# ADVRHumanoids/mpc_fatigue

Hardware: NVIDIA B200
Metric: rollout_steps_per_s_with_jacobians (higher is better)
Workload: dtype f64

## Files before the change

### mpc_fatigue_b200/csrc/kernels_jvp2.cu

```cuda
#include <atomic>
#include <cstdlib>
#include <mutex>
#include <vector>

#include "derivs.cuh"
#include "launch.cuh"

namespace mpcf {

template <int N>
struct WsLayout {
    static constexpr int kTile = 32;
    static constexpr int kPlanes2 = 3 * N * N;
    static constexpr int kPlanes1 = 4 * N;
    static constexpr int kQd = 0, kQdd = N, kFd = 2 * N, kQ = 3 * N;
    static constexpr int kStageDoubles = (kPlanes2 + kPlanes1) * kTile;
    static constexpr unsigned kStageBytes = kStageDoubles * sizeof(double);
    static constexpr int kRingDoubles = (kPlanes2 + 3 * N) * kTile;
    static constexpr unsigned kRingBytes = kRingDoubles * sizeof(double);
    static constexpr int kUnitDoubles = 4 * (kPlanes2 + kPlanes1);
    static MPCF_DI size_t chunk(long tile, int s) { return ((size_t)tile * 4 + s) * kStageDoubles; }
};
size_t jvp_ws_doubles_per_unit(int n) { return (size_t)4 * (3 * n * n + 4 * n); }

template <int N, int L>
__global__ void __launch_bounds__(kThreads) k_step_stages(const __grid_constant__ StaticParams<N> P, long U, long u0, long cnt,
                                                         const double *q, const double *qd, const double *tau, const double *theat,
                                                         long UT, const double *f, double dt, const double *dt_u, double *qn, double *qdn,
                                                         double *fn, double *ws)
{
    static_assert(N == L, "the pipeline runs one serial chain at a time (forests: one launch per chain)");
    const StaticModel<N, L> m{P};
    using D = Dyn<double, StaticModel<N, L>>;
    using W = WsLayout<N>;
    const long lu = (long)blockIdx.x * blockDim.x + threadIdx.x;
    if (lu >= cnt) return;
    const long u = u0 + lu;
    double x[3 * N], t[N], th[N], xs[3 * N], xn[3 * N], k[3 * N];
#pragma unroll
    for (int i = 0; i < N; ++i) {
        x[i] = q[i * U + u];
        x[N + i] = qd[i * U + u];
        x[2 * N + i] = f[i * U + u];
        t[i] = tau[i * U + u];
        th[i] = theat[i * UT + u];
    }
    const double h = dt_u ? dt_u[u] : dt;
#pragma unroll
    for (int i = 0; i < 3 * N; ++i) { xs[i] = x[i]; xn[i] = x[i]; }
#pragma unroll 1
    for (int s = 0; s < 4; ++s) {
        const double cs = s < 2 ? 0.5 : (s == 2 ? 1.0 : 0.0);
        const double wt = (s == 0 || s == 3) ? 1.0 / 6.0 : 1.0 / 3.0;
        double *w = ws + W::chunk(lu / 32, s) + W::kPlanes2 * 32 + (lu & 31);
        {
            double Cs[N * (N + 1) / 2];
            D::template fd_crba<L, true>(m, xs, xs + N, t, k + N, Cs);
#pragma unroll
            for (int i = 0; i < N; ++i) {
                k[i] = xs[N + i];
                k[2 * N + i] = D::fatigue_rhs(m, i, xs[2 * N + i], th[i], xs[N + i]);
            }
            double *c = ws + W::chunk(lu / 32, s) + 2 * N * N * 32 + (lu & 31);
#pragma unroll
            for (int r = 0; r < N; ++r)
#pragma unroll
                for (int cc = 0; cc < N; ++cc) __stcs(c + (r * N + cc) * 32, Cs[r >= cc ? r * (r + 1) / 2 + cc : cc * (cc + 1) / 2 + r]);
        }
#pragma unroll
        for (int i = 0; i < N; ++i) {
            __stcs(w + (W::kQ + i) * 32, xs[i]);
            __stcs(w + (W::kQd + i) * 32, xs[N + i]);
            __stcs(w + (W::kQdd + i) * 32, k[N + i]);
            __stcs(w + (W::kFd + i) * 32, k[2 * N + i]);
        }
        const double a = h * wt, c = h * cs;
#pragma unroll
        for (int i = 0; i < 3 * N; ++i) {
            xn[i] += a * k[i];
            xs[i] = x[i] + c * k[i];
        }
    }
    if (qn) {
#pragma unroll
        for (int i = 0; i < N; ++i) {
            qn[i * U + u] = xn[i];
            qdn[i * U + u] = xn[N + i];
            fn[i * U + u] = xn[2 * N + i];
        }
    }
}

constexpr int kSmCountHint = 148;
MPCF_DI void cp_async8(double *smem, const double *gmem)
{
    asm volatile("cp.async.ca.shared.global [%0], [%1], 8;" ::"r"((unsigned)__cvta_generic_to_shared(smem)), "l"(gmem) : "memory");
}
struct CFromShared {
    double *base;
    int stride;
    MPCF_DI void ready() const { asm volatile("cp.async.commit_group;\n\tcp.async.wait_group 0;" ::: "memory"); }
    MPCF_DI double operator()(int r, int c) const { return base[(r * (r + 1) / 2 + c) * stride]; }
};
template <int N>
struct CFromGlobal {
    const double *o;
    MPCF_DI void ready() const {}
    MPCF_DI double operator()(int r, int c) const { return o[(2 * N * N + r * N + c) * 32]; }
};

template <class F>
struct CFromRegisters {
    F f;
    MPCF_DI void ready() const {}
    MPCF_DI double operator()(int r, int c) const { return f(r, c); }
};

template <int N, int L, bool KSMEM>
__global__ void __launch_bounds__(kThreads) k_stage_derivs(const __grid_constant__ StaticParams<N> P, long cnt, double *ws)
{
    const StaticModel<N, L> m{P};
    using W = WsLayout<N>;
    const long lu = (long)blockIdx.x * blockDim.x + threadIdx.x;
    if (lu >= cnt) return;
    const int s = blockIdx.y;
    double *o = ws + W::chunk(lu / 32, s) + (lu & 31);
    const double *w = o + W::kPlanes2 * 32;
    double q[N], qd[N], qdd[N];
#pragma unroll
    for (int i = 0; i < N; ++i) {
        q[i] = __ldcs(w + (W::kQ + i) * 32);
        qd[i] = __ldcs(w + (W::kQd + i) * 32);
        qdd[i] = __ldcs(w + (W::kQdd + i) * 32);
    }
    {
        const long lin = (long)blockIdx.y * gridDim.x + blockIdx.x + 2 * kSmCountHint;
        if (lin < 4l * gridDim.x) {
            const long lu2 = (lin % gridDim.x) * blockDim.x + threadIdx.x;
            if (lu2 < cnt) {
                const double *o2 = ws + W::chunk(lu2 / 32, (int)(lin / gridDim.x)) + (lu2 & 31);
#pragma unroll
                for (int i = 0; i < N; ++i) {
                    asm volatile("prefetch.global.L2 [%0];" ::"l"(o2 + (W::kPlanes2 + W::kQ + i) * 32));
                    asm volatile("prefetch.global.L2 [%0];" ::"l"(o2 + (W::kPlanes2 + W::kQd + i) * 32));
                    asm volatile("prefetch.global.L2 [%0];" ::"l"(o2 + (W::kPlanes2 + W::kQdd + i) * 32));
                }
#pragma unroll
                for (int r = 0; r < N; ++r)
#pragma unroll
                    for (int c = 0; c <= r; ++c) asm volatile("prefetch.global.L2 [%0];" ::"l"(o2 + (2 * N * N + r * N + c) * 32));
            }
        }
    }
    auto emit = [&](int mat, int r, int c, double v) { __stcs(o + (mat * N * N + r * N + c) * 32, v); };
    if (KSMEM) {
        extern __shared__ double k2_slab[];
        SharedLinkStore ks{k2_slab + threadIdx.x, (int)blockDim.x};
        CFromShared Cs{k2_slab + 18 * (N - 1) * blockDim.x + threadIdx.x, (int)blockDim.x};
#pragma unroll
        for (int r = 0; r < N; ++r)
#pragma unroll
            for (int c = 0; c <= r; ++c) cp_async8(Cs.base + (r * (r + 1) / 2 + c) * Cs.stride, o + (2 * N * N + r * N + c) * 32);
        FdDerivs<StaticModel<N, L>, L>::run_cols(m, q, qd, qdd, Cs, emit, ks);
    } else {
        LocalLinkStore<N> ks;
        CFromGlobal<N> Cs{o};
        FdDerivs<StaticModel<N, L>, L>::run_cols(m, q, qd, qdd, Cs, emit, ks);
    }
}

template <int N>
__global__ void __launch_bounds__(kThreads) k_fd_derivs(const __grid_constant__ StaticParams<N> P, long U, const double *q, const double *qd,
                                                       const double *tau, double *Ao, double *Bo, double *Co, int ntot, int c0)
{
    const StaticModel<N, N> m{P};
    const long u = (long)blockIdx.x * blockDim.x + threadIdx.x;
    if (u >= U) return;
    double a[N], b[N], c[N], qdd[N], Cv[N * (N + 1) / 2];
#pragma unroll
    for (int i = 0; i < N; ++i) { a[i] = q[i * U + u]; b[i] = qd[i * U + u]; c[i] = tau[i * U + u]; }
    Dyn<double, StaticModel<N, N>>::template fd_crba<N, true>(m, a, b, c, qdd, Cv);
    auto at = [&](int r, int cc) { return (size_t)((c0 + r) * ntot + c0 + cc) * U + u; };
#pragma unroll
    for (int r = 0; r < N; ++r)
#pragma unroll
        for (int cc = 0; cc < N; ++cc) Co[at(r, cc)] = Cv[r >= cc ? r * (r + 1) / 2 + cc : cc * (cc + 1) / 2 + r];
    auto cget = [&](int r, int cc) { return Cv[r * (r + 1) / 2 + cc]; };
    CFromRegisters<decltype(cget)> Cs{cget};
    auto emit = [&](int mat, int r, int cc, double v) { (mat == 0 ? Ao : Bo)[at(r, cc)] = v; };
    extern __shared__ double link_slab[];
    SharedLinkStore ks{link_slab + threadIdx.x, (int)blockDim.x};
    FdDerivs<StaticModel<N, N>, N>::run_cols(m, a, b, qdd, Cs, emit, ks);
#pragma unroll 1
    for (int r = 0; r < N; ++r)
#pragma unroll 1
        for (int cc = 0; cc < ntot; ++cc)
            if (cc < c0 || cc >= c0 + N) {
                const size_t k = (size_t)((c0 + r) * ntot + cc) * U + u;
                Ao[k] = 0.0; Bo[k] = 0.0; Co[k] = 0.0;
            }
}

template <int N>
__global__ void __launch_bounds__(kThreads) k_rnea_derivs(const __grid_constant__ StaticParams<N> P, long U, const double *q, const double *qd,
                                                         const double *qdd, double *Dq, double *Dv, double *Mo, int ntot, int c0)
{
    const StaticModel<N, N> m{P};
    const long u = (long)blockIdx.x * blockDim.x + threadIdx.x;
    if (u >= U) return;
    double a[N], b[N], c[N];
#pragma unroll
    for (int i = 0; i < N; ++i) { a[i] = q[i * U + u]; b[i] = qd[i * U + u]; c[i] = qdd ? qdd[i * U + u] : 0.0; }
    extern __shared__ double link_slab[];
    SharedLinkStore ks{link_slab + threadIdx.x, (int)blockDim.x};
    struct Hooks {
        double *Dq, *Dv, *Mo;
        long U, u;
        int ntot, c0;
        MPCF_DI size_t at(int r, int cc) const { return (size_t)((c0 + r) * ntot + c0 + cc) * U + u; }
// ... 108 lines not shown
        for (int cc = 0; cc < ntot; ++cc)
            if (cc < c0 || cc >= c0 + N) { Dq[(size_t)((c0 + r) * ntot + cc) * U + u] = 0.0; Dv[(size_t)((c0 + r) * ntot + cc) * U + u] = 0.0; }
}

struct RneaDerivsDualBody {
    template <class MP>
    static MPCF_DI void run(const MP &m, long u, long U, const double *q, const double *qd, const double *qdd, double *Dq, double *Dv,
                            double *Mo)
    {
        constexpr int UNR = MP::kStatic ? MP::MAXN : 1;
        const int n = m.n();
        const int d = blockIdx.y;
        Dual a[MP::MAXN], b[MP::MAXN], c[MP::MAXN], t[MP::MAXN];
#pragma unroll UNR
        for (int i = 0; i < n; ++i) {
            a[i] = Dual(q[i * U + u], d == i ? 1.0 : 0.0);
            b[i] = Dual(qd[i * U + u], d == n + i ? 1.0 : 0.0);
            c[i] = Dual(qdd ? qdd[i * U + u] : 0.0, d == 2 * n + i ? 1.0 : 0.0);
        }
        Dyn<Dual, MP>::rnea(m, a, b, c, t);
        double *out = d < n ? Dq : (d < 2 * n ? Dv : Mo);
        const int col = d % n;
#pragma unroll UNR
        for (int r = 0; r < n; ++r) out[(size_t)(r * n + col) * U + u] = t[r].d;
    }
};

struct FdDerivsDualBody {
    template <class MP>
    static MPCF_DI void run(const MP &m, long u, long U, const double *q, const double *qd, const double *tau, double *Ao, double *Bo,
                            double *Co)
    {
        constexpr int UNR = MP::kStatic ? MP::MAXN : 1;
        const int n = m.n();
        const int d = blockIdx.y;
        Dual a[MP::MAXN], b[MP::MAXN], c[MP::MAXN], t[MP::MAXN];
#pragma unroll UNR
        for (int i = 0; i < n; ++i) {
            a[i] = Dual(q[i * U + u], d == i ? 1.0 : 0.0);
            b[i] = Dual(qd[i * U + u], d == n + i ? 1.0 : 0.0);
            c[i] = Dual(tau[i * U + u], d == 2 * n + i ? 1.0 : 0.0);
        }
        Dyn<Dual, MP>::aba(m, a, b, c, t);
        double *out = d < n ? Ao : (d < 2 * n ? Bo : Co);
        const int col = d % n;
#pragma unroll UNR
        for (int r = 0; r < n; ++r) out[(size_t)(r * n + col) * U + u] = t[r].d;
    }
};

template <int N, int L>
struct ColumnState {
    double Xq[N], Xv[N], Xf[N], aq[N], av[N], af[N];
    int jq, jv, jt;
    bool isdt;
    double ktau;
    double xq1;

    MPCF_DI void set_tau(const StaticParams<N> &P, double tauj)
    {
        ktau = 0.0;
#pragma unroll
        for (int i = 0; i < N; ++i)
            if (i == jt) ktau = 2.0 * P.fat[i][1] * P.fat[i][2] * tauj;
    }
    MPCF_DI void init(int col)
    {
        jq = col < N ? col : -1;
        jv = (col >= N && col < 2 * N) ? col - N : -1;
        jt = (col >= 2 * N && col < 3 * N) ? col - 2 * N : -1;
        isdt = col == 3 * N;
#pragma unroll
        for (int i = 0; i < N; ++i) {
            Xq[i] = (i == jq) ? 1.0 : 0.0;
            Xv[i] = (i == jv) ? 1.0 : 0.0;
            Xf[i] = 0.0;
            aq[i] = Xq[i]; av[i] = Xv[i]; af[i] = 0.0;
        }
        xq1 = 0.0;
    }
    MPCF_DI void finish(const StaticParams<N> &P, int s, const double *w1, double h, const double *nv)
    {
        const double cs = s < 2 ? 0.5 : (s == 2 ? 1.0 : 0.0);
        const double wt = (s == 0 || s == 3) ? 1.0 / 6.0 : 1.0 / 3.0;
#pragma unroll
        for (int i = 0; i < N; ++i) {
            const double qds = w1[(WsLayout<N>::kQd + i) * 32];
            double kf = 2.0 * P.fat[i][1] * P.fat[i][3] * qds * Xv[i] - P.fat[i][0] * Xf[i];
            if (i == jt) kf += ktau;
            double yq = h * Xv[i], yf = h * kf, yv = h * nv[i];
            if (isdt) {
                yq += qds;
                yv += w1[(WsLayout<N>::kQdd + i) * 32];
                yf += w1[(WsLayout<N>::kFd + i) * 32];
            }
            aq[i] = fma(wt, yq, aq[i]);
            av[i] = fma(wt, yv, av[i]);
            af[i] = fma(wt, yf, af[i]);
            Xq[i] = ((i == jq) ? 1.0 : 0.0) + cs * yq;
            Xv[i] = ((i == jv) ? 1.0 : 0.0) + cs * yv;
            Xf[i] = cs * yf;
            if (s == 0 && (i == jq || i == jv)) xq1 = Xq[i];
        }
    }
    MPCF_DI void stage(const StaticParams<N> &P, int s, const double *w, double h)
    {
        double nv[N];
        if (s == 0) {
#pragma unroll
            for (int r = 0; r < N; ++r) {
                double kv = 0.0;
                if (jq >= 0 && jq / L == r / L) kv = w[(r * N + jq) * 32];
                if (jv >= 0 && jv / L == r / L) kv = w[(N * N + r * N + jv) * 32];
                nv[r] = kv;
            }
        } else if (s == 1 && !isdt) {
            const int js = jq >= 0 ? jq : jv;
#pragma unroll
            for (int r = 0; r < N; ++r) {
                double kv = 0.0;
                if (js >= 0 && js / L == r / L) kv = w[(r * N + js) * 32] * xq1;
#pragma unroll
                for (int c = 0; c < N; ++c) {
                    if (r / L != c / L) continue;
                    kv = fma(w[(N * N + r * N + c) * 32], Xv[c], kv);
                }
                nv[r] = kv;
            }
        } else {
#pragma unroll
            for (int r = 0; r < N; ++r) {
                double kv = 0.0;
#pragma unroll
                for (int c = 0; c < N; ++c) {
                    if (r / L != c / L) continue;
                    kv = fma(w[(r * N + c) * 32], Xq[c], kv);
                    kv = fma(w[(N * N + r * N + c) * 32], Xv[c], kv);
                }
                nv[r] = kv;
            }
        }
        if (jt >= 0) {
#pragma unroll
            for (int r = 0; r < N; ++r)
                if (jt / L == r / L) nv[r] += w[(2 * N * N + r * N + jt) * 32];
        }
        finish(P, s, w + 3 * N * N * 32, h, nv);
    }
    static MPCF_DI void stage2(ColumnState &a, ColumnState &b, const StaticParams<N> &P, int s, const double *w, double h)
    {
        double na[N], nb[N];
#pragma unroll
        for (int r = 0; r < N; ++r) {
            double ka = 0.0, kb = 0.0;
#pragma unroll
            for (int c = 0; c < N; ++c) {
                if (r / L != c / L) continue;
                const double A = w[(r * N + c) * 32], B = w[(N * N + r * N + c) * 32];
                ka = fma(A, a.Xq[c], ka);
                kb = fma(A, b.Xq[c], kb);
                ka = fma(B, a.Xv[c], ka);
                kb = fma(B, b.Xv[c], kb);
            }
            if (a.jt >= 0 && a.jt / L == r / L) ka += w[(2 * N * N + r * N + a.jt) * 32];
            if (b.jt >= 0 && b.jt / L == r / L) kb += w[(2 * N * N + r * N + b.jt) * 32];
            na[r] = ka;
            nb[r] = kb;
        }
        a.finish(P, s, w + 3 * N * N * 32, h, na);
        b.finish(P, s, w + 3 * N * N * 32, h, nb);
    }
    template <bool WHOLE>
    MPCF_DI void store(const StaticParams<N> &P, int col, double h, long U, long u, double *jac, int ntot_, int c0_) const
    {
        const int ntot = WHOLE ? N : ntot_, c0 = WHOLE ? 0 : c0_;
        const long PC = 4 * ntot + 1;
        const long ocol = isdt ? 4 * ntot : (col / N) * ntot + c0 + col % N;
#pragma unroll
        for (int i = 0; i < N; ++i) {
            __stcs(jac + ((size_t)(c0 + i) * PC + ocol) * U + u, aq[i]);
            __stcs(jac + ((size_t)(ntot + c0 + i) * PC + ocol) * U + u, av[i]);
            __stcs(jac + ((size_t)(2 * ntot + c0 + i) * PC + ocol) * U + u, af[i]);
        }
        if (isdt) {
#pragma unroll
            for (int j = 0; j < N; ++j) {
                const double z = P.fat[j][0] * h;
                const double g = 1.0 + z * (-1.0 + z * (0.5 + z * (-1.0 / 6.0 + z * (1.0 / 24.0))));
                if (WHOLE) {
#pragma unroll
                    for (int r = 0; r < 3 * N; ++r) __stcs(jac + ((size_t)r * PC + 3 * N + j) * U + u, (r == 2 * N + j) ? g : 0.0);
                } else {
#pragma unroll
                    for (int blk = 0; blk < 3; ++blk)
#pragma unroll
                        for (int i = 0; i < N; ++i)
                            __stcs(jac + ((size_t)(blk * ntot + c0 + i) * PC + 3 * ntot + c0 + j) * U + u, (blk == 2 && i == j) ? g : 0.0);
                }
            }
        }
    }
};

MPCF_DI unsigned smem_u32(const void *p) { return (unsigned)__cvta_generic_to_shared(p); }
MPCF_DI void mbar_init(unsigned long long *bar, unsigned count)
{
    asm volatile("mbarrier.init.shared::cta.b64 [%0], %1;" ::"r"(smem_u32(bar)), "r"(count) : "memory");
}
MPCF_DI void mbar_arrive(unsigned long long *bar)
{
    asm volatile("{\n\t.reg .b64 st;\n\tmbarrier.arrive.shared::cta.b64 st, [%0];\n\t}" ::"r"(smem_u32(bar)) : "memory");
}
MPCF_DI void mbar_arrive_expect_tx(unsigned long long *bar, unsigned bytes)
{
    asm volatile("{\n\t.reg .b64 st;\n\tmbarrier.arrive.expect_tx.release.cta.shared::cta.b64 st, [%0], %1;\n\t}" ::"r"(smem_u32(bar)), "r"(bytes)
                 : "memory");
}
MPCF_DI void mbar_wait(unsigned long long *bar, unsigned parity)
{
    unsigned done;
    do {
        asm volatile("{\n\t.reg .pred p;\n\tmbarrier.try_wait.parity.shared::cta.b64 p, [%1], %2;\n\tselp.b32 %0, 1, 0, p;\n\t}"
                     : "=r"(done)
                     : "r"(smem_u32(bar)), "r"(parity)
                     : "memory");
    } while (!done);
}
MPCF_DI void bulk_g2s(void *dst, const void *src, unsigned bytes, unsigned long long *bar)
{
    asm volatile("cp.async.bulk.shared::cluster.global.mbarrier::complete_tx::bytes [%0], [%1], %2, [%3];" ::"r"(smem_u32(dst)), "l"(src),
                 "r"(bytes), "r"(smem_u32(bar))
                 : "memory");
}

template <class W, int NBUF>
MPCF_DI void tma_issue(unsigned item, double *buf, unsigned long long *full, unsigned long long *empty, const double *ws, unsigned bid,
                       unsigned nblk)
{
    const unsigned slot = item % NBUF, round = item / NBUF;
    const long t = bid + (long)(item / 4) * nblk;
    mbar_wait(&empty[slot], (round & 1) ^ 1);
    mbar_arrive_expect_tx(&full[slot], W::kRingBytes);
    bulk_g2s(buf + (size_t)slot * W::kRingDoubles, ws + W::chunk(t, item & 3), W::kRingBytes, &full[slot]);
}

template <int N, int L, int NBUF, int CPW, bool WHOLE>
__global__ void __launch_bounds__(32 * ((3 * N + CPW) / CPW), 1)
    k_chain_rule_tma(const __grid_constant__ StaticParams<N> P, long U, long u0, long cnt, const double *__restrict__ tau, long UT, double dt,
                     const double *__restrict__ dt_u, const double *__restrict__ ws, double *__restrict__ jac, long UJ, int ntot, int c0)
{
    using W = WsLayout<N>;
    constexpr int NC = 3 * N + 1;
    constexpr int NW = (NC + CPW - 1) / CPW;
    extern __shared__ __align__(128) unsigned char smem_raw[];
    double *buf = reinterpret_cast<double *>(smem_raw);
    unsigned long long *full = reinterpret_cast<unsigned long long *>(smem_raw + (size_t)NBUF * W::kRingBytes);
    unsigned long long *empty = full + NBUF;
    const int warp = threadIdx.x >> 5, lane = threadIdx.x & 31;
    const long ntiles = (cnt + 31) / 32;
    const long my_tiles = blockIdx.x < ntiles ? (ntiles - blockIdx.x + gridDim.x - 1) / gridDim.x : 0;
    const unsigned nitems = (unsigned)(my_tiles * 4);
    const bool producer = threadIdx.x == 0;
    if (producer) {
        for (int i = 0; i < NBUF; ++i) { mbar_init(&full[i], 1); mbar_init(&empty[i], NW); }
        asm volatile("fence.mbarrier_init.release.cluster;" ::: "memory");
        for (unsigned i = 0; i < NBUF - 1 && i < nitems; ++i)
            tma_issue<W, NBUF>(i, buf, full, empty, ws, blockIdx.x, gridDim.x);
    }
    __syncthreads();
    const int col0 = warp, col1 = warp + NW;
    const bool two = CPW == 2 && col1 < NC;
    unsigned it = 0;
    for (long t = blockIdx.x; t < ntiles; t += gridDim.x) {
        const long lu = t * 32 + lane;
        const bool live = lu < cnt;
        const long u = u0 + (live ? lu : 0);
        const double h = dt_u ? dt_u[u] : dt;
        ColumnState<N, L> a, b;
        a.init(col0);
        a.set_tau(P, a.jt >= 0 ? tau[(size_t)a.jt * UT + u] : 0.0);
        if (CPW == 2) {
            b.init(two ? col1 : col0);
            b.set_tau(P, b.jt >= 0 ? tau[(size_t)b.jt * UT + u] : 0.0);
        }
#pragma unroll 1
        for (int s = 0; s < 4; ++s, ++it) {
            if (producer && it + NBUF - 1 < nitems) tma_issue<W, NBUF>(it + NBUF - 1, buf, full, empty, ws, blockIdx.x, gridDim.x);
            const unsigned slot = it % NBUF, round = it / NBUF;
            mbar_wait(&full[slot], round & 1);
            const double *w = buf + (size_t)slot * W::kRingDoubles + lane;
            if (CPW == 2) ColumnState<N, L>::stage2(a, b, P, s, w, h);
            else a.stage(P, s, w, h);
            __syncwarp();
            if (lane == 0) mbar_arrive(&empty[slot]);
        }
        if (live) {
            a.template store<WHOLE>(P, col0, h, UJ, u, jac, ntot, c0);
            if (two) b.template store<WHOLE>(P, col1, h, UJ, u, jac, ntot, c0);
        }
    }
}

template <int N, int L, int NCY>
__global__ void __launch_bounds__(32 * NCY, 2)
    k_chain_rule_ldg(const __grid_constant__ StaticParams<N> P, long U, long u0, long cnt, const double *__restrict__ tau, long UT, double dt,
                     const double *__restrict__ dt_u, const double *__restrict__ ws, double *__restrict__ jac, long UJ, int ntot, int c0)
{
    using W = WsLayout<N>;
    const long lu = (long)blockIdx.x * 32 + threadIdx.x;
    if (lu >= cnt) return;
    const long u = u0 + lu;
    const double h = dt_u ? dt_u[u] : dt;
    constexpr int NC = 3 * N + 1;
    for (int col = threadIdx.y; col < NC; col += blockDim.y) {
        ColumnState<N, L> st;
        st.init(col);
        st.set_tau(P, st.jt >= 0 ? tau[(size_t)st.jt * UT + u] : 0.0);
#pragma unroll 1
        for (int s = 0; s < 4; ++s) st.stage(P, s, ws + W::chunk(blockIdx.x, s) + threadIdx.x, h);
        st.template store<false>(P, col, h, UJ, u, jac, ntot, c0);
    }
}

struct ProfEvent { cudaEvent_t a, b; int k; };
static std::atomic<bool> g_prof_on{false};
static std::mutex g_prof_mu;
static std::vector<ProfEvent> g_prof;
void jvp_profile_enable(bool on) { g_prof_on.store(on); }
static cudaEvent_t prof_begin(int k, cudaStream_t s)
{
    if (!g_prof_on.load(std::memory_order_relaxed)) return nullptr;
    ProfEvent e;
    cudaEventCreate(&e.a);
    cudaEventCreate(&e.b);
    e.k = k;
    cudaEventRecord(e.a, s);
    std::lock_guard<std::mutex> lk(g_prof_mu);
    g_prof.push_back(e);
    return e.b;
}
static void prof_end(cudaEvent_t b, cudaStream_t s)
{
    if (b) cudaEventRecord(b, s);
}
int jvp_profile_read(double *ms3, long *launches)
{
    std::lock_guard<std::mutex> lk(g_prof_mu);
    ms3[0] = ms3[1] = ms3[2] = 0.0;
    *launches = (long)g_prof.size();
    for (auto &e : g_prof) {
        float t = 0.f;
        cudaEventSynchronize(e.b);
        cudaEventElapsedTime(&t, e.a, e.b);
        ms3[e.k] += t;
        cudaEventDestroy(e.a);
        cudaEventDestroy(e.b);
    }
    g_prof.clear();
    return 0;
}

static int current_device()
{
    int dev = 0;
    cudaGetDevice(&dev);
    return dev >= 0 && dev < 64 ? dev : 0;
}
static int sm_count()
{
    static int n[64] = {};
    const int dev = current_device();
    if (!n[dev]) {
        cudaDeviceGetAttribute(&n[dev], cudaDevAttrMultiProcessorCount, dev);
        if (n[dev] <= 0) n[dev] = 148;
    }
    return n[dev];
}

template <int N, int L>
static cudaError_t run_jvp2(const StaticParams<N> &P, long U, long Ucnt, const double *q, const double *qd, const double *tau, const double *theat,
                            long UT, const double *f,
                            double dt, const double *dt_u, double *qn, double *qdn, double *fn, double *jac, long UJ, double *ws, long Uc,
                            cudaStream_t s, int ntot = N, int c0 = 0)
{
    using W = WsLayout<N>;
    constexpr bool kTma = N <= 7;
    constexpr int kRingMax = (227 * 1024 - 256) / (int)W::kRingBytes;
    constexpr int NBUF = kTma ? (kRingMax > 5 ? 5 : kRingMax) : 0;
    constexpr int kCpwDefault = (3 * N + 1 <= 19) ? 1 : 2;
    constexpr size_t smem = (size_t)NBUF * W::kRingBytes + 2 * NBUF * sizeof(unsigned long long);
    constexpr int kK2Threads = (2 * (18 * (N - 1) + N * (N + 1) / 2) * kThreads * (int)sizeof(double) <= 227 * 1024) ? kThreads : 96;
    constexpr int kK2Slab = (18 * (N - 1) + N * (N + 1) / 2) * kK2Threads * (int)sizeof(double);
    constexpr bool kK2Smem = N == L && 2 * kK2Slab <= 227 * 1024;
    if constexpr (kTma) {
        static std::atomic<bool> attr_set[64];
        const int dev = current_device();
        if (!attr_set[dev].load(std::memory_order_acquire)) {
            cudaError_t e = cudaSuccess;
            if constexpr (kCpwDefault == 1) {
                e = cudaFuncSetAttribute(k_chain_rule_tma<N, L, NBUF, 1, true>, cudaFuncAttributeMaxDynamicSharedMemorySize, (int)smem);
                if (e != cudaSuccess) return e;
                e = cudaFuncSetAttribute(k_chain_rule_tma<N, L, NBUF, 1, false>, cudaFuncAttributeMaxDynamicSharedMemorySize, (int)smem);
                if (e != cudaSuccess) return e;
            }
            e = cudaFuncSetAttribute(k_chain_rule_tma<N, L, NBUF, 2, true>, cudaFuncAttributeMaxDynamicSharedMemorySize, (int)smem);
            if (e != cudaSuccess) return e;
            e = cudaFuncSetAttribute(k_chain_rule_tma<N, L, NBUF, 2, false>, cudaFuncAttributeMaxDynamicSharedMemorySize, (int)smem);
            if (e != cudaSuccess) return e;
            if constexpr (kK2Smem) {
                e = cudaFuncSetAttribute(k_stage_derivs<N, L, true>, cudaFuncAttributeMaxDynamicSharedMemorySize, kK2Slab);
                if (e != cudaSuccess) return e;
            }
            attr_set[dev].store(true, std::memory_order_release);
        }
    }
    for (long u0 = 0; u0 < Ucnt; u0 += Uc) {
        const long cnt = (Ucnt - u0) < Uc ? (Ucnt - u0) : Uc;
        const unsigned gb = (unsigned)((cnt + kThreads - 1) / kThreads);
        const long ntiles = (cnt + 31) / 32;
        cudaEvent_t pe = prof_begin(0, s);
        k_step_stages<N, L><<<gb, kThreads, 0, s>>>(P, U, u0, cnt, q, qd, tau, theat, UT, f, dt, dt_u, qn, qdn, fn, ws);
        prof_end(pe, s);
        pe = prof_begin(1, s);
        static const int k2smem = getenv("MPCF_K2_SMEM") ? atoi(getenv("MPCF_K2_SMEM")) : 1;
        bool k2done = false;
        if constexpr (kK2Smem) {
            if (k2smem) {
                k_stage_derivs<N, L, true><<<dim3((unsigned)((cnt + kK2Threads - 1) / kK2Threads), 4), kK2Threads, kK2Slab, s>>>(P, cnt, ws);
                k2done = true;
            }
        }
        if (!k2done) k_stage_derivs<N, L, false><<<dim3(gb, 4), kThreads, 0, s>>>(P, cnt, ws);
        prof_end(pe, s);
        pe = prof_begin(2, s);
        if constexpr (kTma) {
            const unsigned g3 = (unsigned)(ntiles < sm_count() ? ntiles : sm_count());
            static const int cpw_env = getenv("MPCF_K3_CPW") ? atoi(getenv("MPCF_K3_CPW")) : 1;
            const int cpw = kCpwDefault == 2 ? 2 : cpw_env;
            if (cpw == 2) {
                (ntot == N ? k_chain_rule_tma<N, L, NBUF, 2, true> : k_chain_rule_tma<N, L, NBUF, 2, false>)<<<g3, 32 * ((3 * N + 2) / 2), smem, s>>>(
                    P, U, u0, cnt, theat, UT, dt, dt_u, ws, jac, UJ, ntot, c0);
            } else if constexpr (kCpwDefault == 1) {
                (ntot == N ? k_chain_rule_tma<N, L, NBUF, 1, true> : k_chain_rule_tma<N, L, NBUF, 1, false>)<<<g3, 32 * (3 * N + 1), smem, s>>>(
                    P, U, u0, cnt, theat, UT, dt, dt_u, ws, jac, UJ, ntot, c0);
            }
        } else {
            k_chain_rule_ldg<N, L, 10><<<(unsigned)ntiles, dim3(32, 10), 0, s>>>(P, U, u0, cnt, theat, UT, dt, dt_u, ws, jac, UJ, ntot, c0);
        }
        prof_end(pe, s);
        g_launches.fetch_add(3);
    }
    return cudaGetLastError();
}

template <int L, class V>
__global__ void __launch_bounds__(256) k_forest_fill_cross(int ntot, long cntv, long UJ, double *jac)
{
    const long uv = (long)blockIdx.x * blockDim.x + threadIdx.x;
    if (uv >= cntv) return;
    const int r = blockIdx.y, rc = (r % ntot) / L, nch = ntot / L;
    const long PC = 4 * ntot + 1;
    V zero;
    memset(&zero, 0, sizeof(V));
    double *row = jac + (size_t)r * PC * UJ;
    for (int b = 0; b < 4; ++b)
        for (int oc = 0; oc < nch; ++oc) {
            if (oc == rc) continue;
            double *p = row + (size_t)(b * ntot + oc * L) * UJ;
#pragma unroll
            for (int i = 0; i < L; ++i) __stcs(reinterpret_cast<V *>(p + (size_t)i * UJ) + uv, zero);
        }
}

template <int L>
static cudaError_t run_forest(const LaunchModel &m, long U, long Ucnt, const double *q, const double *qd, const double *tau, const double *theat,
                              long UT, const double *f, double dt,
                              const double *dt_u, double *qn, double *qdn, double *fn, double *jac, long UJ, double *ws, long Uc, cudaStream_t s)
{
    const StaticParams<L> *cp = static_cast<const StaticParams<L> *>(m.chain_params);
    for (int c = 0; c < m.n / L; ++c) {
        const size_t off = (size_t)c * L * U;
        cudaError_t e = run_jvp2<L, L>(cp[c], U, Ucnt, q + off, qd + off, tau + off, theat + (size_t)c * L * UT, UT, f + off, dt, dt_u, qn ? qn + off : nullptr,
                                       qdn ? qdn + off : nullptr, fn ? fn + off : nullptr, jac, UJ, ws, Uc, s, m.n, L * c);
        if (e != cudaSuccess) return e;
    }
    if (Ucnt % 2 == 0 && UJ % 2 == 0 && (reinterpret_cast<size_t>(jac) & 15) == 0)
        k_forest_fill_cross<L, double2><<<dim3((unsigned)((Ucnt / 2 + 255) / 256), 3 * m.n), 256, 0, s>>>(m.n, Ucnt / 2, UJ, jac);
    else
        k_forest_fill_cross<L, double><<<dim3((unsigned)((Ucnt + 255) / 256), 3 * m.n), 256, 0, s>>>(m.n, Ucnt, UJ, jac);
    g_launches.fetch_add(1);
    return cudaGetLastError();
}

bool jvp2_supported(const LaunchModel &m) { return family_chain_len(m.fam) > 0; }

cudaError_t launch_step_jvp_ws(const LaunchModel &m, long U, const double *q, const double *qd, const double *tau, const double *f,
                               double dt, const double *dt_u, double *qn, double *qdn, double *fn, double *jac, double *ws,
                               size_t ws_bytes, cudaStream_t s, long cnt, long UJ, const double *theat, long UT)
// ... 120 lines not shown
```

Baseline: 230.2 million.

## Swizzle workspace planes and stage Jacobian stores through shared memory

Adds an XOR swizzle on the per-tile workspace planes so lanes reading several planes from the shared-memory ring hit different banks, and routes all workspace accesses through the new layout. For one-column-per-warp chain-rule kernels it adds a specialised flat stage path plus a padded shared staging buffer with named barriers, so Jacobian outputs are transposed and written coalesced. The column-per-warp choice becomes compile-time by N, dropping the environment switch. This trades ring capacity for staging memory and adds barrier synchronisation among the worker warps.

```diff
diff --git a/mpc_fatigue_b200/csrc/kernels_jvp2.cu b/mpc_fatigue_b200/csrc/kernels_jvp2.cu
--- a/mpc_fatigue_b200/csrc/kernels_jvp2.cu
+++ b/mpc_fatigue_b200/csrc/kernels_jvp2.cu
@@ -1,6 +1,7 @@
 #include <atomic>
 #include <cstdlib>
 #include <mutex>
+#include <type_traits>
 #include <vector>
 
 #include "derivs.cuh"
@@ -20,6 +21,20 @@
     static constexpr unsigned kRingBytes = kRingDoubles * sizeof(double);
     static constexpr int kUnitDoubles = 4 * (kPlanes2 + kPlanes1);
     static MPCF_DI size_t chunk(long tile, int s) { return ((size_t)tile * 4 + s) * kStageDoubles; }
+    static MPCF_HD int swz(int plane) { return 4 * (plane % 3); }
+    static MPCF_HD int at(int plane, int u) { return plane * kTile + (u ^ swz(plane)); }
+};
+
+template <int N>
+struct WsView {
+    const double *b0, *b1, *b2;
+    MPCF_DI WsView(const double *chunk, int u) : b0(chunk + u), b1(chunk + (u ^ 4)), b2(chunk + (u ^ 8)) {}
+    MPCF_DI const double *ptr(int P) const
+    {
+        const int k = P % 3;
+        return (k == 0 ? b0 : (k == 1 ? b1 : b2)) + P * WsLayout<N>::kTile;
+    }
+    MPCF_DI double operator[](int P) const { return *ptr(P); }
 };
 size_t jvp_ws_doubles_per_unit(int n) { return (size_t)4 * (3 * n * n + 4 * n); }
 
@@ -52,7 +67,8 @@
     for (int s = 0; s < 4; ++s) {
         const double cs = s < 2 ? 0.5 : (s == 2 ? 1.0 : 0.0);
         const double wt = (s == 0 || s == 3) ? 1.0 / 6.0 : 1.0 / 3.0;
-        double *w = ws + W::chunk(lu / 32, s) + W::kPlanes2 * 32 + (lu & 31);
+        double *w = ws + W::chunk(lu / 32, s);
+        const int uu = (int)(lu & 31);
         {
             double Cs[N * (N + 1) / 2];
             D::template fd_crba<L, true>(m, xs, xs + N, t, k + N, Cs);
@@ -61,18 +77,18 @@
                 k[i] = xs[N + i];
                 k[2 * N + i] = D::fatigue_rhs(m, i, xs[2 * N + i], th[i], xs[N + i]);
             }
-            double *c = ws + W::chunk(lu / 32, s) + 2 * N * N * 32 + (lu & 31);
 #pragma unroll
             for (int r = 0; r < N; ++r)
 #pragma unroll
-                for (int cc = 0; cc < N; ++cc) __stcs(c + (r * N + cc) * 32, Cs[r >= cc ? r * (r + 1) / 2 + cc : cc * (cc + 1) / 2 + r]);
+                for (int cc = 0; cc < N; ++cc)
+                    __stcs(w + W::at(2 * N * N + r * N + cc, uu), Cs[r >= cc ? r * (r + 1) / 2 + cc : cc * (cc + 1) / 2 + r]);
         }
 #pragma unroll
         for (int i = 0; i < N; ++i) {
-            __stcs(w + (W::kQ + i) * 32, xs[i]);
-            __stcs(w + (W::kQd + i) * 32, xs[N + i]);
-            __stcs(w + (W::kQdd + i) * 32, k[N + i]);
-            __stcs(w + (W::kFd + i) * 32, k[2 * N + i]);
+            __stcs(w + W::at(W::kPlanes2 + W::kQ + i, uu), xs[i]);
+            __stcs(w + W::at(W::kPlanes2 + W::kQd + i, uu), xs[N + i]);
+            __stcs(w + W::at(W::kPlanes2 + W::kQdd + i, uu), k[N + i]);
+            __stcs(w + W::at(W::kPlanes2 + W::kFd + i, uu), k[2 * N + i]);
         }
         const double a = h * wt, c = h * cs;
 #pragma unroll
@@ -105,8 +121,9 @@
 template <int N>
 struct CFromGlobal {
     const double *o;
+    int u;
     MPCF_DI void ready() const {}
-    MPCF_DI double operator()(int r, int c) const { return o[(2 * N * N + r * N + c) * 32]; }
+    MPCF_DI double operator()(int r, int c) const { return o[WsLayout<N>::at(2 * N * N + r * N + c, u)]; }
 };
 
 template <class F>
@@ -124,35 +141,36 @@
     const long lu = (long)blockIdx.x * blockDim.x + threadIdx.x;
     if (lu >= cnt) return;
     const int s = blockIdx.y;
-    double *o = ws + W::chunk(lu / 32, s) + (lu & 31);
-    const double *w = o + W::kPlanes2 * 32;
+    double *o = ws + W::chunk(lu / 32, s);
+    const int uu = (int)(lu & 31);
     double q[N], qd[N], qdd[N];
 #pragma unroll
     for (int i = 0; i < N; ++i) {
-        q[i] = __ldcs(w + (W::kQ + i) * 32);
-        qd[i] = __ldcs(w + (W::kQd + i) * 32);
-        qdd[i] = __ldcs(w + (W::kQdd + i) * 32);
+        q[i] = __ldcs(o + W::at(W::kPlanes2 + W::kQ + i, uu));
+        qd[i] = __ldcs(o + W::at(W::kPlanes2 + W::kQd + i, uu));
+        qdd[i] = __ldcs(o + W::at(W::kPlanes2 + W::kQdd + i, uu));
     }
     {
         const long lin = (long)blockIdx.y * gridDim.x + blockIdx.x + 2 * kSmCountHint;
         if (lin < 4l * gridDim.x) {
             const long lu2 = (lin % gridDim.x) * blockDim.x + threadIdx.x;
             if (lu2 < cnt) {
-                const double *o2 = ws + W::chunk(lu2 / 32, (int)(lin / gridDim.x)) + (lu2 & 31);
+                const double *o2 = ws + W::chunk(lu2 / 32, (int)(lin / gridDim.x));
+                const int u2 = (int)(lu2 & 31);
 #pragma unroll
                 for (int i = 0; i < N; ++i) {
-                    asm volatile("prefetch.global.L2 [%0];" ::"l"(o2 + (W::kPlanes2 + W::kQ + i) * 32));
-                    asm volatile("prefetch.global.L2 [%0];" ::"l"(o2 + (W::kPlanes2 + W::kQd + i) * 32));
-                    asm volatile("prefetch.global.L2 [%0];" ::"l"(o2 + (W::kPlanes2 + W::kQdd + i) * 32));
+                    asm volatile("prefetch.global.L2 [%0];" ::"l"(o2 + W::at(W::kPlanes2 + W::kQ + i, u2)));
+                    asm volatile("prefetch.global.L2 [%0];" ::"l"(o2 + W::at(W::kPlanes2 + W::kQd + i, u2)));
+                    asm volatile("prefetch.global.L2 [%0];" ::"l"(o2 + W::at(W::kPlanes2 + W::kQdd + i, u2)));
                 }
 #pragma unroll
                 for (int r = 0; r < N; ++r)
 #pragma unroll
-                    for (int c = 0; c <= r; ++c) asm volatile("prefetch.global.L2 [%0];" ::"l"(o2 + (2 * N * N + r * N + c) * 32));
-            }
-        }
-    }
-    auto emit = [&](int mat, int r, int c, double v) { __stcs(o + (mat * N * N + r * N + c) * 32, v); };
+                    for (int c = 0; c <= r; ++c) asm volatile("prefetch.global.L2 [%0];" ::"l"(o2 + W::at(2 * N * N + r * N + c, u2)));
+            }
+        }
+    }
+    auto emit = [&](int mat, int r, int c, double v) { __stcs(o + W::at(mat * N * N + r * N + c, uu), v); };
     if (KSMEM) {
         extern __shared__ double k2_slab[];
         SharedLinkStore ks{k2_slab + threadIdx.x, (int)blockDim.x};
@@ -160,11 +178,11 @@
 #pragma unroll
         for (int r = 0; r < N; ++r)
 #pragma unroll
-            for (int c = 0; c <= r; ++c) cp_async8(Cs.base + (r * (r + 1) / 2 + c) * Cs.stride, o + (2 * N * N + r * N + c) * 32);
+            for (int c = 0; c <= r; ++c) cp_async8(Cs.base + (r * (r + 1) / 2 + c) * Cs.stride, o + W::at(2 * N * N + r * N + c, uu));
         FdDerivs<StaticModel<N, L>, L>::run_cols(m, q, qd, qdd, Cs, emit, ks);
     } else {
         LocalLinkStore<N> ks;
-        CFromGlobal<N> Cs{o};
+        CFromGlobal<N> Cs{o, uu};
         FdDerivs<StaticModel<N, L>, L>::run_cols(m, q, qd, qdd, Cs, emit, ks);
     }
 }
@@ -379,78 +397,78 @@
 template <int N, int L>
 struct ColumnState {
     double Xq[N], Xv[N], Xf[N], aq[N], av[N], af[N];
-    int jq, jv, jt;
-    bool isdt;
-    double ktau;
-    double xq1;
+    int col;
+    MPCF_DI int jq() const { return col < N ? col : -1; }
+    MPCF_DI int jv() const { return (col >= N && col < 2 * N) ? col - N : -1; }
+    MPCF_DI int jt() const { return (col >= 2 * N && col < 3 * N) ? col - 2 * N : -1; }
+    MPCF_DI bool isdt() const { return col == 3 * N; }
+    double aux;
 
     MPCF_DI void set_tau(const StaticParams<N> &P, double tauj)
     {
-        ktau = 0.0;
+        aux = 0.0;
 #pragma unroll
         for (int i = 0; i < N; ++i)
-            if (i == jt) ktau = 2.0 * P.fat[i][1] * P.fat[i][2] * tauj;
-    }
-    MPCF_DI void init(int col)
-    {
-        jq = col < N ? col : -1;
-        jv = (col >= N && col < 2 * N) ? col - N : -1;
-        jt = (col >= 2 * N && col < 3 * N) ? col - 2 * N : -1;
-        isdt = col == 3 * N;
+            if (i == jt()) aux = 2.0 * P.fat[i][1] * P.fat[i][2] * tauj;
+    }
+    MPCF_DI void init(int c)
+    {
+        col = c;
 #pragma unroll
         for (int i = 0; i < N; ++i) {
-            Xq[i] = (i == jq) ? 1.0 : 0.0;
-            Xv[i] = (i == jv) ? 1.0 : 0.0;
+            Xq[i] = (i == jq()) ? 1.0 : 0.0;
+            Xv[i] = (i == jv()) ? 1.0 : 0.0;
             Xf[i] = 0.0;
             aq[i] = Xq[i]; av[i] = Xv[i]; af[i] = 0.0;
         }
-        xq1 = 0.0;
-    }
-    MPCF_DI void finish(const StaticParams<N> &P, int s, const double *w1, double h, const double *nv)
-    {
+    }
+    template <bool NODT = false>
+    MPCF_DI void finish(const StaticParams<N> &P, int s, const WsView<N> &w, double h, const double *nv)
+    {
+        using W = WsLayout<N>;
         const double cs = s < 2 ? 0.5 : (s == 2 ? 1.0 : 0.0);
         const double wt = (s == 0 || s == 3) ? 1.0 / 6.0 : 1.0 / 3.0;
 #pragma unroll
         for (int i = 0; i < N; ++i) {
-            const double qds = w1[(WsLayout<N>::kQd + i) * 32];
+            const double qds = w[W::kPlanes2 + W::kQd + i];
             double kf = 2.0 * P.fat[i][1] * P.fat[i][3] * qds * Xv[i] - P.fat[i][0] * Xf[i];
-            if (i == jt) kf += ktau;
+            if (i == jt()) kf += aux;
             double yq = h * Xv[i], yf = h * kf, yv = h * nv[i];
-            if (isdt) {
+            if (!NODT && isdt()) {
                 yq += qds;
-                yv += w1[(WsLayout<N>::kQdd + i) * 32];
-                yf += w1[(WsLayout<N>::kFd + i) * 32];
+                yv += w[W::kPlanes2 + W::kQdd + i];
+                yf += w[W::kPlanes2 + W::kFd + i];
             }
             aq[i] = fma(wt, yq, aq[i]);
             av[i] = fma(wt, yv, av[i]);
             af[i] = fma(wt, yf, af[i]);
-            Xq[i] = ((i == jq) ? 1.0 : 0.0) + cs * yq;
-            Xv[i] = ((i == jv) ? 1.0 : 0.0) + cs * yv;
+            Xq[i] = ((i == jq()) ? 1.0 : 0.0) + cs * yq;
+            Xv[i] = ((i == jv()) ? 1.0 : 0.0) + cs * yv;
             Xf[i] = cs * yf;
-            if (s == 0 && (i == jq || i == jv)) xq1 = Xq[i];
-        }
-    }
-    MPCF_DI void stage(const StaticParams<N> &P, int s, const double *w, double h)
+            if (s == 0 && (i == jq() || i == jv())) aux = Xq[i];
+        }
+    }
+    MPCF_DI void stage(const StaticParams<N> &P, int s, const WsView<N> &w, double h)
     {
         double nv[N];
         if (s == 0) {
 #pragma unroll
             for (int r = 0; r < N; ++r) {
                 double kv = 0.0;
-                if (jq >= 0 && jq / L == r / L) kv = w[(r * N + jq) * 32];
-                if (jv >= 0 && jv / L == r / L) kv = w[(N * N + r * N + jv) * 32];
+                if (jq() >= 0 && jq() / L == r / L) kv = w[r * N + jq()];
+                if (jv() >= 0 && jv() / L == r / L) kv = w[N * N + r * N + jv()];
                 nv[r] = kv;
             }
-        } else if (s == 1 && !isdt) {
-            const int js = jq >= 0 ? jq : jv;
+        } else if (s == 1 && !isdt()) {
+            const int js = jq() >= 0 ? jq() : jv();
 #pragma unroll
             for (int r = 0; r < N; ++r) {
                 double kv = 0.0;
-                if (js >= 0 && js / L == r / L) kv = w[(r * N + js) * 32] * xq1;
+                if (js >= 0 && js / L == r / L) kv = w[r * N + js] * aux;
 #pragma unroll
                 for (int c = 0; c < N; ++c) {
                     if (r / L != c / L) continue;
-                    kv = fma(w[(N * N + r * N + c) * 32], Xv[c], kv);
+                    kv = fma(w[N * N + r * N + c], Xv[c], kv);
                 }
                 nv[r] = kv;
             }
@@ -461,20 +479,63 @@
 #pragma unroll
                 for (int c = 0; c < N; ++c) {
                     if (r / L != c / L) continue;
-                    kv = fma(w[(r * N + c) * 32], Xq[c], kv);
-                    kv = fma(w[(N * N + r * N + c) * 32], Xv[c], kv);
+                    kv = fma(w[r * N + c], Xq[c], kv);
+                    kv = fma(w[N * N + r * N + c], Xv[c], kv);
                 }
                 nv[r] = kv;
             }
         }
-        if (jt >= 0) {
+        if (jt() >= 0) {
 #pragma unroll
             for (int r = 0; r < N; ++r)
-                if (jt / L == r / L) nv[r] += w[(2 * N * N + r * N + jt) * 32];
-        }
-        finish(P, s, w + 3 * N * N * 32, h, nv);
-    }
-    static MPCF_DI void stage2(ColumnState &a, ColumnState &b, const StaticParams<N> &P, int s, const double *w, double h)
+                if (jt() / L == r / L) nv[r] += w[2 * N * N + r * N + jt()];
+        }
+        finish(P, s, w, h, nv);
+    }
+    MPCF_DI void stage_flat(const StaticParams<N> &P, int s, const double *slot, const WsView<N> &w, int lpA, double h)
+    {
+        static_assert(N == L && N % 3 == 0, "one serial chain with a plane count per row that keeps the swizzle class");
+        constexpr int T = WsLayout<N>::kTile, RS = N * T;
+        const int lp0 = lpA + (col / N) * (N * N * T), lpC = lpA + 2 * N * N * T;
+        const bool istau = jt() >= 0;
+        double nv[N];
+        if (s == 0) {
+#pragma unroll
+            for (int r = 0; r < N; ++r) {
+                const double e = slot[lp0 + r * RS];
+                nv[r] = istau ? 0.0 + e : e;
+            }
+        } else {
+            if (s == 1) {
+#pragma unroll
+                for (int r = 0; r < N; ++r) {
+                    const double e = slot[lpA + r * RS];
+                    double kv = istau ? 0.0 : e * aux;
+#pragma unroll
+                    for (int c = 0; c < N; ++c) kv = fma(w[N * N + r * N + c], Xv[c], kv);
+                    nv[r] = kv;
+                }
+            } else {
+#pragma unroll
+                for (int r = 0; r < N; ++r) {
+                    double kv = 0.0;
+#pragma unroll
+                    for (int c = 0; c < N; ++c) {
+                        kv = fma(w[r * N + c], Xq[c], kv);
+                        kv = fma(w[N * N + r * N + c], Xv[c], kv);
+                    }
+                    nv[r] = kv;
+                }
+            }
+#pragma unroll
+            for (int r = 0; r < N; ++r) {
+                const double e = istau ? slot[lpC + r * RS] : 0.0;
+                nv[r] = istau ? nv[r] + e : nv[r];
+            }
+        }
+        finish<true>(P, s, w, h, nv);
+    }
+    static MPCF_DI void stage2(ColumnState &a, ColumnState &b, const StaticParams<N> &P, int s, const WsView<N> &w, double h)
     {
         double na[N], nb[N];
 #pragma unroll
@@ -483,33 +544,33 @@
 #pragma unroll
             for (int c = 0; c < N; ++c) {
                 if (r / L != c / L) continue;
-                const double A = w[(r * N + c) * 32], B = w[(N * N + r * N + c) * 32];
+                const double A = w[r * N + c], B = w[N * N + r * N + c];
                 ka = fma(A, a.Xq[c], ka);
                 kb = fma(A, b.Xq[c], kb);
                 ka = fma(B, a.Xv[c], ka);
                 kb = fma(B, b.Xv[c], kb);
             }
-            if (a.jt >= 0 && a.jt / L == r / L) ka += w[(2 * N * N + r * N + a.jt) * 32];
-            if (b.jt >= 0 && b.jt / L == r / L) kb += w[(2 * N * N + r * N + b.jt) * 32];
+            if (a.jt() >= 0 && a.jt() / L == r / L) ka += w[2 * N * N + r * N + a.jt()];
+            if (b.jt() >= 0 && b.jt() / L == r / L) kb += w[2 * N * N + r * N + b.jt()];
             na[r] = ka;
             nb[r] = kb;
         }
-        a.finish(P, s, w + 3 * N * N * 32, h, na);
-        b.finish(P, s, w + 3 * N * N * 32, h, nb);
+        a.finish(P, s, w, h, na);
+        b.finish(P, s, w, h, nb);
     }
     template <bool WHOLE>
     MPCF_DI void store(const StaticParams<N> &P, int col, double h, long U, long u, double *jac, int ntot_, int c0_) const
     {
         const int ntot = WHOLE ? N : ntot_, c0 = WHOLE ? 0 : c0_;
         const long PC = 4 * ntot + 1;
-        const long ocol = isdt ? 4 * ntot : (col / N) * ntot + c0 + col % N;
+        const long ocol = isdt() ? 4 * ntot : (col / N) * ntot + c0 + col % N;
 #pragma unroll
         for (int i = 0; i < N; ++i) {
             __stcs(jac + ((size_t)(c0 + i) * PC + ocol) * U + u, aq[i]);
             __stcs(jac + ((size_t)(ntot + c0 + i) * PC + ocol) * U + u, av[i]);
             __stcs(jac + ((size_t)(2 * ntot + c0 + i) * PC + ocol) * U + u, af[i]);
         }
-        if (isdt) {
+        if (isdt()) {
 #pragma unroll
             for (int j = 0; j < N; ++j) {
                 const double z = P.fat[j][0] * h;
@@ -571,6 +632,14 @@
     bulk_g2s(buf + (size_t)slot * W::kRingDoubles, ws + W::chunk(t, item & 3), W::kRingBytes, &full[slot]);
 }
 
+template <int N>
+struct JacStage {
+    static constexpr int kPitch = 33;
+    static constexpr int kDoubles = N * 3 * N * kPitch;
+};
+
+MPCF_DI void named_bar_sync(int id, int threads) { asm volatile("bar.sync %0, %1;" ::"r"(id), "r"(threads) : "memory"); }
+
 template <int N, int L, int NBUF, int CPW, bool WHOLE>
 __global__ void __launch_bounds__(32 * ((3 * N + CPW) / CPW), 1)
     k_chain_rule_tma(const __grid_constant__ StaticParams<N> P, long U, long u0, long cnt, const double *__restrict__ tau, long UT, double dt,
@@ -579,9 +648,10 @@
     using W = WsLayout<N>;
     constexpr int NC = 3 * N + 1;
     constexpr int NW = (NC + CPW - 1) / CPW;
+    constexpr size_t kStgBytes = CPW == 1 ? JacStage<N>::kDoubles * sizeof(double) : 0;
     extern __shared__ __align__(128) unsigned char smem_raw[];
     double *buf = reinterpret_cast<double *>(smem_raw);
-    unsigned long long *full = reinterpret_cast<unsigned long long *>(smem_raw + (size_t)NBUF * W::kRingBytes);
+    unsigned long long *full = reinterpret_cast<unsigned long long *>(smem_raw + (size_t)NBUF * W::kRingBytes + kStgBytes);
     unsigned long long *empty = full + NBUF;
     const int warp = threadIdx.x >> 5, lane = threadIdx.x & 31;
     const long ntiles = (cnt + 31) / 32;
@@ -595,35 +665,87 @@
             tma_issue<W, NBUF>(i, buf, full, empty, ws, blockIdx.x, gridDim.x);
     }
     __syncthreads();
-    const int col0 = warp, col1 = warp + NW;
-    const bool two = CPW == 2 && col1 < NC;
     unsigned it = 0;
-    for (long t = blockIdx.x; t < ntiles; t += gridDim.x) {
-        const long lu = t * 32 + lane;
-        const bool live = lu < cnt;
-        const long u = u0 + (live ? lu : 0);
-        const double h = dt_u ? dt_u[u] : dt;
-        ColumnState<N, L> a, b;
-        a.init(col0);
-        a.set_tau(P, a.jt >= 0 ? tau[(size_t)a.jt * UT + u] : 0.0);
-        if (CPW == 2) {
+    if constexpr (CPW == 1) {
+        constexpr int NF = 3 * N;
+        constexpr int SP = JacStage<N>::kPitch;
+        double *stg = buf + (size_t)NBUF * W::kRingDoubles;
+        auto tiles = [&](auto dt_warp) {
+            constexpr bool DTW = decltype(dt_warp)::value;
+            const int uo = DTW ? lane : (int)threadIdx.x / NF;
+            const int col = DTW ? NF : (int)threadIdx.x % NF;
+            const int j = col % N;
+            const int lpA = W::at(j, uo);
+            for (long t = blockIdx.x; t < ntiles; t += gridDim.x) {
+                const long lu = t * 32 + uo;
+                const bool live = lu < cnt;
+                const long u = u0 + (live ? lu : 0);
+                const double h = dt_u ? dt_u[u] : dt;
+                ColumnState<N, L> a;
+                a.init(col);
+                a.set_tau(P, a.jt() >= 0 ? tau[(size_t)a.jt() * UT + u] : 0.0);
+#pragma unroll 1
+                for (int s = 0; s < 4; ++s, ++it) {
+                    if (producer && it + NBUF - 1 < nitems) tma_issue<W, NBUF>(it + NBUF - 1, buf, full, empty, ws, blockIdx.x, gridDim.x);
+                    const unsigned slot = it % NBUF, round = it / NBUF;
+                    mbar_wait(&full[slot], round & 1);
+                    const double *w = buf + (size_t)slot * W::kRingDoubles;
+                    if (DTW) a.stage(P, s, WsView<N>(w, uo), h);
+                    else a.stage_flat(P, s, w, WsView<N>(w, uo), lpA, h);
+                    __syncwarp();
+                    if (lane == 0) mbar_arrive(&empty[slot]);
+                }
+                if (DTW) {
+                    if (live) a.template store<WHOLE>(P, col, h, UJ, u, jac, ntot, c0);
+                    continue;
+                }
+                const int nt = WHOLE ? N : ntot, cz = WHOLE ? 0 : c0;
+                const int PC = 4 * nt + 1;
+                const int ocol = (warp / N) * nt + cz + warp % N;
+                const bool out = t * 32 + lane < cnt;
+                double *dst = jac + (u0 + t * 32 + lane);
+#pragma unroll
+                for (int blk = 0; blk < 3; ++blk) {
+                    named_bar_sync(1, 32 * NF);
+#pragma unroll
+                    for (int i = 0; i < N; ++i) stg[(i * NF + a.col) * SP + uo] = blk == 0 ? a.aq[i] : (blk == 1 ? a.av[i] : a.af[i]);
+                    named_bar_sync(1, 32 * NF);
+#pragma unroll
+                    for (int i = 0; i < N; ++i) {
+                        const double x = stg[(i * NF + warp) * SP + lane];
+                        if (out) __stcs(dst + ((size_t)(blk * nt + cz + i) * PC + ocol) * UJ, x);
+                    }
+                }
+            }
+        };
+        if (warp == NF) tiles(std::true_type{});
+        else tiles(std::false_type{});
+    } else {
+        const int col0 = warp, col1 = warp + NW;
+        const bool two = col1 < NC;
+        for (long t = blockIdx.x; t < ntiles; t += gridDim.x) {
+            const long lu = t * 32 + lane;
+            const bool live = lu < cnt;
+            const long u = u0 + (live ? lu : 0);
+            const double h = dt_u ? dt_u[u] : dt;
+            ColumnState<N, L> a, b;
+            a.init(col0);
+            a.set_tau(P, a.jt() >= 0 ? tau[(size_t)a.jt() * UT + u] : 0.0);
             b.init(two ? col1 : col0);
-            b.set_tau(P, b.jt >= 0 ? tau[(size_t)b.jt * UT + u] : 0.0);
-        }
+            b.set_tau(P, b.jt() >= 0 ? tau[(size_t)b.jt() * UT + u] : 0.0);
 #pragma unroll 1
-        for (int s = 0; s < 4; ++s, ++it) {
-            if (producer && it + NBUF - 1 < nitems) tma_issue<W, NBUF>(it + NBUF - 1, buf, full, empty, ws, blockIdx.x, gridDim.x);
-            const unsigned slot = it % NBUF, round = it / NBUF;
-            mbar_wait(&full[slot], round & 1);
-            const double *w = buf + (size_t)slot * W::kRingDoubles + lane;
-            if (CPW == 2) ColumnState<N, L>::stage2(a, b, P, s, w, h);
-            else a.stage(P, s, w, h);
-            __syncwarp();
-            if (lane == 0) mbar_arrive(&empty[slot]);
-        }
-        if (live) {
-            a.template store<WHOLE>(P, col0, h, UJ, u, jac, ntot, c0);
-            if (two) b.template store<WHOLE>(P, col1, h, UJ, u, jac, ntot, c0);
+            for (int s = 0; s < 4; ++s, ++it) {
+                if (producer && it + NBUF - 1 < nitems) tma_issue<W, NBUF>(it + NBUF - 1, buf, full, empty, ws, blockIdx.x, gridDim.x);
+                const unsigned slot = it % NBUF, round = it / NBUF;
+                mbar_wait(&full[slot], round & 1);
+                ColumnState<N, L>::stage2(a, b, P, s, WsView<N>(buf + (size_t)slot * W::kRingDoubles, lane), h);
+                __syncwarp();
+                if (lane == 0) mbar_arrive(&empty[slot]);
+            }
+            if (live) {
+                a.template store<WHOLE>(P, col0, h, UJ, u, jac, ntot, c0);
+                if (two) b.template store<WHOLE>(P, col1, h, UJ, u, jac, ntot, c0);
+            }
         }
     }
 }
@@ -642,9 +764,9 @@
     for (int col = threadIdx.y; col < NC; col += blockDim.y) {
         ColumnState<N, L> st;
         st.init(col);
-        st.set_tau(P, st.jt >= 0 ? tau[(size_t)st.jt * UT + u] : 0.0);
+        st.set_tau(P, st.jt() >= 0 ? tau[(size_t)st.jt() * UT + u] : 0.0);
 #pragma unroll 1
-        for (int s = 0; s < 4; ++s) st.stage(P, s, ws + W::chunk(blockIdx.x, s) + threadIdx.x, h);
+        for (int s = 0; s < 4; ++s) st.stage(P, s, WsView<N>(ws + W::chunk(blockIdx.x, s), threadIdx.x), h);
         st.template store<false>(P, col, h, UJ, u, jac, ntot, c0);
     }
 }
@@ -712,10 +834,11 @@
 {
     using W = WsLayout<N>;
     constexpr bool kTma = N <= 7;
-    constexpr int kRingMax = (227 * 1024 - 256) / (int)W::kRingBytes;
+    constexpr int kCpw = N <= 6 ? 1 : 2;
+    constexpr size_t kStgBytes = kCpw == 1 ? JacStage<N>::kDoubles * sizeof(double) : 0;
+    constexpr int kRingMax = (int)((227 * 1024 - 256 - kStgBytes) / W::kRingBytes);
     constexpr int NBUF = kTma ? (kRingMax > 5 ? 5 : kRingMax) : 0;
-    constexpr int kCpwDefault = (3 * N + 1 <= 19) ? 1 : 2;
-    constexpr size_t smem = (size_t)NBUF * W::kRingBytes + 2 * NBUF * sizeof(unsigned long long);
+    constexpr size_t smem = (size_t)NBUF * W::kRingBytes + kStgBytes + 2 * NBUF * sizeof(unsigned long long);
     constexpr int kK2Threads = (2 * (18 * (N - 1) + N * (N + 1) / 2) * kThreads * (int)sizeof(double) <= 227 * 1024) ? kThreads : 96;
     constexpr int kK2Slab = (18 * (N - 1) + N * (N + 1) / 2) * kK2Threads * (int)sizeof(double);
     constexpr bool kK2Smem = N == L && 2 * kK2Slab <= 227 * 1024;
@@ -723,16 +846,9 @@
         static std::atomic<bool> attr_set[64];
         const int dev = current_device();
         if (!attr_set[dev].load(std::memory_order_acquire)) {
-            cudaError_t e = cudaSuccess;
-            if constexpr (kCpwDefault == 1) {
-                e = cudaFuncSetAttribute(k_chain_rule_tma<N, L, NBUF, 1, true>, cudaFuncAttributeMaxDynamicSharedMemorySize, (int)smem);
-                if (e != cudaSuccess) return e;
-                e = cudaFuncSetAttribute(k_chain_rule_tma<N, L, NBUF, 1, false>, cudaFuncAttributeMaxDynamicSharedMemorySize, (int)smem);
-                if (e != cudaSuccess) return e;
-            }
-            e = cudaFuncSetAttribute(k_chain_rule_tma<N, L, NBUF, 2, true>, cudaFuncAttributeMaxDynamicSharedMemorySize, (int)smem);
+            cudaError_t e = cudaFuncSetAttribute(k_chain_rule_tma<N, L, NBUF, kCpw, true>, cudaFuncAttributeMaxDynamicSharedMemorySize, (int)smem);
             if (e != cudaSuccess) return e;
-            e = cudaFuncSetAttribute(k_chain_rule_tma<N, L, NBUF, 2, false>, cudaFuncAttributeMaxDynamicSharedMemorySize, (int)smem);
+            e = cudaFuncSetAttribute(k_chain_rule_tma<N, L, NBUF, kCpw, false>, cudaFuncAttributeMaxDynamicSharedMemorySize, (int)smem);
             if (e != cudaSuccess) return e;
             if constexpr (kK2Smem) {
                 e = cudaFuncSetAttribute(k_stage_derivs<N, L, true>, cudaFuncAttributeMaxDynamicSharedMemorySize, kK2Slab);
@@ -762,15 +878,8 @@
         pe = prof_begin(2, s);
         if constexpr (kTma) {
             const unsigned g3 = (unsigned)(ntiles < sm_count() ? ntiles : sm_count());
-            static const int cpw_env = getenv("MPCF_K3_CPW") ? atoi(getenv("MPCF_K3_CPW")) : 1;
-            const int cpw = kCpwDefault == 2 ? 2 : cpw_env;
-            if (cpw == 2) {
-                (ntot == N ? k_chain_rule_tma<N, L, NBUF, 2, true> : k_chain_rule_tma<N, L, NBUF, 2, false>)<<<g3, 32 * ((3 * N + 2) / 2), smem, s>>>(
-                    P, U, u0, cnt, theat, UT, dt, dt_u, ws, jac, UJ, ntot, c0);
-            } else if constexpr (kCpwDefault == 1) {
-                (ntot == N ? k_chain_rule_tma<N, L, NBUF, 1, true> : k_chain_rule_tma<N, L, NBUF, 1, false>)<<<g3, 32 * (3 * N + 1), smem, s>>>(
-                    P, U, u0, cnt, theat, UT, dt, dt_u, ws, jac, UJ, ntot, c0);
-            }
+            (ntot == N ? k_chain_rule_tma<N, L, NBUF, kCpw, true> : k_chain_rule_tma<N, L, NBUF, kCpw, false>)<<<g3, 32 * ((3 * N + kCpw) / kCpw), smem, s>>>(
+                P, U, u0, cnt, theat, UT, dt, dt_u, ws, jac, UJ, ntot, c0);
         } else {
             k_chain_rule_ldg<N, L, 10><<<(unsigned)ntiles, dim3(32, 10), 0, s>>>(P, U, u0, cnt, theat, UT, dt, dt_u, ws, jac, UJ, ntot, c0);
         }
```

Result: slower. 197.9 million (median of 6 runs) (-14.0%).
